# facebookresearch/multimodal

Hardware: NVIDIA H100
Metric: image-text pairs/sec (CLIP ViT-B/16 contrastive pretrain step, bs=512/GPU) (higher is better)
Workload: dtype bf16

## Files before the change

### multimodal_b200/csrc/common.cuh

```cuda
#pragma once
#include <cuda.h>
#include <cuda_bf16.h>
#include <cuda_runtime.h>
#include <stdint.h>
#include <stdio.h>

namespace mmb {

__device__ __forceinline__ uint32_t smem_u32(const void* p) {
  return static_cast<uint32_t>(__cvta_generic_to_shared(p));
}

__device__ __forceinline__ uint64_t global_timer_ns() {
  uint64_t t;
  asm volatile("mov.u64 %0, %%globaltimer;" : "=l"(t));
  return t;
}

#ifndef MMB_WATCHDOG_NS
#define MMB_WATCHDOG_NS 4000000000ull
#endif

__device__ __forceinline__ void mbar_init(uint64_t* bar, uint32_t count) {
  asm volatile("mbarrier.init.shared::cta.b64 [%0], %1;" ::"r"(smem_u32(bar)), "r"(count) : "memory");
// ... 25 lines not shown
      : "=r"(ok)
      : "r"(smem_u32(bar)), "r"(parity)
      : "memory");
  return ok != 0;
}
__device__ __forceinline__ void mbar_wait(uint64_t* bar, uint32_t parity) {
  if (mbar_try_wait(bar, parity)) return;
  uint32_t polls = 0;
  uint64_t t0 = 0;
  while (!mbar_try_wait(bar, parity)) {
#ifdef MMB_WAIT_NANOSLEEP
    __nanosleep(MMB_WAIT_NANOSLEEP);
#endif
    if ((++polls & 1023u) == 0) {
      const uint64_t now = global_timer_ns();
      if (t0 == 0) t0 = now;
      else if (now - t0 > MMB_WATCHDOG_NS) {
        printf("mmb watchdog: mbarrier wait timed out (block %d thread %d parity %u)\n", (int)blockIdx.x,
               (int)threadIdx.x, parity);
        __trap();
      }
    }
  }
}

__device__ __forceinline__ void mbar_wait_quiet(uint64_t* bar, uint32_t parity) {
  if (mbar_try_wait(bar, parity)) return;
  uint32_t polls = 0;
  uint64_t t0 = 0;
  while (!mbar_try_wait(bar, parity)) {
    if ((++polls & 1023u) == 0) {
      const uint64_t now = global_timer_ns();
      if (t0 == 0) t0 = now;
      else if (now - t0 > MMB_WATCHDOG_NS) __trap();
    }
  }
}

__device__ __forceinline__ void tma_prefetch_desc(const CUtensorMap* m) {
  asm volatile("prefetch.tensormap [%0];" ::"l"(reinterpret_cast<uint64_t>(m)) : "memory");
}
__device__ __forceinline__ void tma_prefetch_l2_2d(const CUtensorMap* m, int c0, int c1) {
  asm volatile("cp.async.bulk.prefetch.tensor.2d.L2.global.tile [%0, {%1, %2}];" ::"l"(reinterpret_cast<uint64_t>(m)),
               "r"(c0), "r"(c1)
               : "memory");
}
__device__ __forceinline__ void tma_load_2d(const CUtensorMap* m, uint64_t* bar, void* smem, int c0, int c1) {
  asm volatile(
      "cp.async.bulk.tensor.2d.shared::cluster.global.mbarrier::complete_tx::bytes [%0], [%1, {%3, %4}], [%2];"
      ::"r"(smem_u32(smem)), "l"(reinterpret_cast<uint64_t>(m)), "r"(smem_u32(bar)), "r"(c0), "r"(c1)
      : "memory");
}
__device__ __forceinline__ void tma_load_3d(const CUtensorMap* m, uint64_t* bar, void* smem, int c0, int c1,
                                            int c2) {
  asm volatile(
      "cp.async.bulk.tensor.3d.shared::cluster.global.mbarrier::complete_tx::bytes [%0], [%1, {%3, %4, %5}], [%2];"
      ::"r"(smem_u32(smem)), "l"(reinterpret_cast<uint64_t>(m)), "r"(smem_u32(bar)), "r"(c0), "r"(c1), "r"(c2)
      : "memory");
}
__device__ __forceinline__ void tma_store_2d(const CUtensorMap* m, const void* smem, int c0, int c1) {
  asm volatile("cp.async.bulk.tensor.2d.global.shared::cta.bulk_group [%0, {%2, %3}], [%1];" ::"l"(
                   reinterpret_cast<uint64_t>(m)),
               "r"(smem_u32(smem)), "r"(c0), "r"(c1)
               : "memory");
}
__device__ __forceinline__ void tma_store_3d(const CUtensorMap* m, const void* smem, int c0, int c1, int c2) {
  asm volatile("cp.async.bulk.tensor.3d.global.shared::cta.bulk_group [%0, {%2, %3, %4}], [%1];" ::"l"(
                   reinterpret_cast<uint64_t>(m)),
               "r"(smem_u32(smem)), "r"(c0), "r"(c1), "r"(c2)
               : "memory");
}
__device__ __forceinline__ void tma_reduce_add_2d(const CUtensorMap* m, const void* smem, int c0, int c1) {
  asm volatile("cp.reduce.async.bulk.tensor.2d.global.shared::cta.add.bulk_group [%0, {%2, %3}], [%1];" ::"l"(
                   reinterpret_cast<uint64_t>(m)),
               "r"(smem_u32(smem)), "r"(c0), "r"(c1)
               : "memory");
}
__device__ __forceinline__ void tma_store_commit() { asm volatile("cp.async.bulk.commit_group;" ::: "memory"); }
template <int N>
__device__ __forceinline__ void tma_store_wait_read() {
  asm volatile("cp.async.bulk.wait_group.read %0;" ::"n"(N) : "memory");
}
template <int N>
__device__ __forceinline__ void tma_store_wait_all() {
  asm volatile("cp.async.bulk.wait_group %0;" ::"n"(N) : "memory");
}

__device__ __forceinline__ uint32_t cluster_ctarank() {
  uint32_t r;
  asm volatile("mov.u32 %0, %%cluster_ctarank;" : "=r"(r));
  return r;
}
__device__ __forceinline__ void cluster_sync_all() {
  asm volatile("barrier.cluster.arrive.release.aligned;\n\tbarrier.cluster.wait.acquire.aligned;" ::: "memory");
}
__device__ __forceinline__ void tma_load_2d_multicast(const CUtensorMap* m, uint64_t* bar, void* smem, int c0, int c1,
                                                      uint16_t cta_mask) {
  asm volatile(
      "cp.async.bulk.tensor.2d.shared::cluster.global.mbarrier::complete_tx::bytes.multicast::cluster [%0], [%1, {%3, "
      "%4}], [%2], %5;" ::"r"(smem_u32(smem)),
      "l"(reinterpret_cast<uint64_t>(m)), "r"(smem_u32(bar)), "r"(c0), "r"(c1), "h"(cta_mask)
      : "memory");
}

__device__ __forceinline__ uint64_t make_smem_desc_sw128(uint32_t saddr, uint32_t lbo_bytes, uint32_t sbo_bytes) {
  uint64_t d = 0;
  d |= (uint64_t)((saddr & 0x3FFFFu) >> 4);
  d |= (uint64_t)((lbo_bytes >> 4) & 0x3FFFu) << 16;
  d |= (uint64_t)((sbo_bytes >> 4) & 0x3FFFu) << 32;
  d |= (uint64_t)1 << 62;
  return d;
}
__device__ __forceinline__ void wgmma_fence() { asm volatile("wgmma.fence.sync.aligned;" ::: "memory"); }
__device__ __forceinline__ void wgmma_commit() { asm volatile("wgmma.commit_group.sync.aligned;" ::: "memory"); }
template <int N>
__device__ __forceinline__ void wgmma_wait() {
  asm volatile("wgmma.wait_group.sync.aligned %0;" ::"n"(N) : "memory");
}
template <int TA, int TB>
__device__ __forceinline__ void wgmma_m64n256k16(float (&d)[128], uint64_t adesc, uint64_t bdesc, uint32_t accumulate) {
  asm volatile(
      "{\n\t.reg .pred p;\n\t"
      "setp.ne.b32 p, %130, 0;\n\t"
      "wgmma.mma_async.sync.aligned.m64n256k16.f32.bf16.bf16 "
      "{"
      "%0, %1, %2, %3, %4, %5, %6, %7, %8, %9, %10, %11, %12, %13, %14, %15, "
      "%16, %17, %18, %19, %20, %21, %22, %23, %24, %25, %26, %27, %28, %29, %30, %31, "
      "%32, %33, %34, %35, %36, %37, %38, %39, %40, %41, %42, %43, %44, %45, %46, %47, "
      "%48, %49, %50, %51, %52, %53, %54, %55, %56, %57, %58, %59, %60, %61, %62, %63, "
      "%64, %65, %66, %67, %68, %69, %70, %71, %72, %73, %74, %75, %76, %77, %78, %79, "
      "%80, %81, %82, %83, %84, %85, %86, %87, %88, %89, %90, %91, %92, %93, %94, %95, "
      "%96, %97, %98, %99, %100, %101, %102, %103, %104, %105, %106, %107, %108, %109, %110, %111, "
      "%112, %113, %114, %115, %116, %117, %118, %119, %120, %121, %122, %123, %124, %125, %126, %127"
      "}, %128, %129, p, 1, 1, %131, %132;\n\t}"
      : "+f"(d[0]), "+f"(d[1]), "+f"(d[2]), "+f"(d[3]), "+f"(d[4]), "+f"(d[5]), "+f"(d[6]), "+f"(d[7]),
        "+f"(d[8]), "+f"(d[9]), "+f"(d[10]), "+f"(d[11]), "+f"(d[12]), "+f"(d[13]), "+f"(d[14]), "+f"(d[15]),
        "+f"(d[16]), "+f"(d[17]), "+f"(d[18]), "+f"(d[19]), "+f"(d[20]), "+f"(d[21]), "+f"(d[22]), "+f"(d[23]),
        "+f"(d[24]), "+f"(d[25]), "+f"(d[26]), "+f"(d[27]), "+f"(d[28]), "+f"(d[29]), "+f"(d[30]), "+f"(d[31]),
        "+f"(d[32]), "+f"(d[33]), "+f"(d[34]), "+f"(d[35]), "+f"(d[36]), "+f"(d[37]), "+f"(d[38]), "+f"(d[39]),
        "+f"(d[40]), "+f"(d[41]), "+f"(d[42]), "+f"(d[43]), "+f"(d[44]), "+f"(d[45]), "+f"(d[46]), "+f"(d[47]),
        "+f"(d[48]), "+f"(d[49]), "+f"(d[50]), "+f"(d[51]), "+f"(d[52]), "+f"(d[53]), "+f"(d[54]), "+f"(d[55]),
        "+f"(d[56]), "+f"(d[57]), "+f"(d[58]), "+f"(d[59]), "+f"(d[60]), "+f"(d[61]), "+f"(d[62]), "+f"(d[63]),
        "+f"(d[64]), "+f"(d[65]), "+f"(d[66]), "+f"(d[67]), "+f"(d[68]), "+f"(d[69]), "+f"(d[70]), "+f"(d[71]),
        "+f"(d[72]), "+f"(d[73]), "+f"(d[74]), "+f"(d[75]), "+f"(d[76]), "+f"(d[77]), "+f"(d[78]), "+f"(d[79]),
        "+f"(d[80]), "+f"(d[81]), "+f"(d[82]), "+f"(d[83]), "+f"(d[84]), "+f"(d[85]), "+f"(d[86]), "+f"(d[87]),
        "+f"(d[88]), "+f"(d[89]), "+f"(d[90]), "+f"(d[91]), "+f"(d[92]), "+f"(d[93]), "+f"(d[94]), "+f"(d[95]),
        "+f"(d[96]), "+f"(d[97]), "+f"(d[98]), "+f"(d[99]), "+f"(d[100]), "+f"(d[101]), "+f"(d[102]), "+f"(d[103]),
        "+f"(d[104]), "+f"(d[105]), "+f"(d[106]), "+f"(d[107]), "+f"(d[108]), "+f"(d[109]), "+f"(d[110]), "+f"(d[111]),
        "+f"(d[112]), "+f"(d[113]), "+f"(d[114]), "+f"(d[115]), "+f"(d[116]), "+f"(d[117]), "+f"(d[118]), "+f"(d[119]),
        "+f"(d[120]), "+f"(d[121]), "+f"(d[122]), "+f"(d[123]), "+f"(d[124]), "+f"(d[125]), "+f"(d[126]), "+f"(d[127])
      : "l"(adesc), "l"(bdesc), "r"(accumulate), "n"(TA), "n"(TB));
}

template <int N>
__device__ __forceinline__ void setmaxnreg_dec() { asm volatile("setmaxnreg.dec.sync.aligned.u32 %0;" ::"n"(N)); }
template <int N>
__device__ __forceinline__ void setmaxnreg_inc() { asm volatile("setmaxnreg.inc.sync.aligned.u32 %0;" ::"n"(N)); }

__device__ __forceinline__ void ldsm_x4(uint32_t (&r)[4], uint32_t addr) {
  asm volatile("ldmatrix.sync.aligned.m8n8.x4.shared.b16 {%0,%1,%2,%3}, [%4];"
               : "=r"(r[0]), "=r"(r[1]), "=r"(r[2]), "=r"(r[3])
               : "r"(addr));
}
__device__ __forceinline__ void ldsm_x4_t(uint32_t (&r)[4], uint32_t addr) {
  asm volatile("ldmatrix.sync.aligned.m8n8.x4.trans.shared.b16 {%0,%1,%2,%3}, [%4];"
               : "=r"(r[0]), "=r"(r[1]), "=r"(r[2]), "=r"(r[3])
               : "r"(addr));
}
__device__ __forceinline__ void mma16816(float (&d)[4], const uint32_t (&a)[4], uint32_t b0, uint32_t b1) {
  asm volatile(
      "mma.sync.aligned.m16n8k16.row.col.f32.bf16.bf16.f32 {%0,%1,%2,%3}, {%4,%5,%6,%7}, {%8,%9}, {%0,%1,%2,%3};"
      : "+f"(d[0]), "+f"(d[1]), "+f"(d[2]), "+f"(d[3])
      : "r"(a[0]), "r"(a[1]), "r"(a[2]), "r"(a[3]), "r"(b0), "r"(b1));
}

__device__ __forceinline__ uint32_t pack_bf16x2(float lo, float hi) {
  __nv_bfloat162 v = __floats2bfloat162_rn(lo, hi);
  return *reinterpret_cast<uint32_t*>(&v);
}
__device__ __forceinline__ float bf16_lo(uint32_t v) { return __uint_as_float(v << 16); }
__device__ __forceinline__ float bf16_hi(uint32_t v) { return __uint_as_float(v & 0xFFFF0000u); }

__device__ __forceinline__ float ex2_approx(float x) {
  float y;
  asm("ex2.approx.ftz.f32 %0, %1;" : "=f"(y) : "f"(x));
  return y;
}
__device__ __forceinline__ float rcp_approx(float x) {
  float y;
  asm("rcp.approx.ftz.f32 %0, %1;" : "=f"(y) : "f"(x));
  return y;
}
__device__ __forceinline__ float fast_sigmoid(float z) {
  return rcp_approx(1.f + ex2_approx(-1.4426950408889634f * z));
}
__device__ __forceinline__ float tanh_approx(float x) {
  float y;
  asm("tanh.approx.f32 %0, %1;" : "=f"(y) : "f"(x));
  return y;
}
__device__ __forceinline__ float quick_gelu(float x) {
  const float t = tanh_approx(0.851f * x), h = 0.5f * x;
  return fmaf(h, t, h);
}
__device__ __forceinline__ float quick_gelu_grad(float x) {
  const float u = 0.851f * x;
  const float t = tanh_approx(u);
  return fmaf(0.5f, fmaf(u, fmaf(-t, t, 1.f), t), 0.5f);
}
__device__ __forceinline__ float gelu_erf(float x) { return 0.5f * x * (1.f + erff(x * 0.70710678118654752f)); }
__device__ __forceinline__ float gelu_erf_grad(float x) {
  return 0.5f * (1.f + erff(x * 0.70710678118654752f)) + x * 0.3989422804014327f * ex2_approx(-0.7213475204444817f * x * x);
}
template <int ACT>
__device__ __forceinline__ float act_fn(float x) { return ACT == 0 ? quick_gelu(x) : gelu_erf(x); }
template <int ACT>
__device__ __forceinline__ float act_grad(float x) { return ACT == 0 ? quick_gelu_grad(x) : gelu_erf_grad(x); }

}
```

### multimodal_b200/csrc/gemm.cu

```cuda
#include "common.cuh"
#include "mmb200_internal.h"
#include <stdlib.h>
#include <mutex>

namespace mmb {

constexpr int BLOCK_M = 128;
constexpr int BLOCK_N = 256;
constexpr int BLOCK_K = 64;
constexpr int WG_K = 16;
constexpr int STAGES = 4;
constexpr int A_BYTES = BLOCK_M * BLOCK_K * 2;
constexpr int B_BYTES = BLOCK_N * BLOCK_K * 2;
constexpr int GEMM_THREADS = 384;
constexpr int STG_BYTES = 64 * 128;
constexpr int EPI_SMEM = 4 * STG_BYTES;
constexpr int GEMM_SMEM_BYTES = 1024  + STAGES * (A_BYTES + B_BYTES) + EPI_SMEM + 256 ;
static_assert(GEMM_SMEM_BYTES <= 227 * 1024, "H100: at most 227 KB of shared memory per block");

struct GemmArgs {
  int M, N, K;
  int m_tiles, n_tiles, splits, kb_total, kb_per_split;
  float alpha;
  const float* bias;
// ... 244 lines not shown
            wg_bar_sync(cw);
#pragma unroll
            for (int jj = 0; jj < 4; ++jj) {
              const int j = 4 * q + jj;
              const int n = nq + 8 * j;
              float b0 = 0.f, b1 = 0.f;
              if (add_bias && n < p.N) { b0 = __ldg(p.bias + n); b1 = __ldg(p.bias + n + 1); }
#pragma unroll
              for (int i = 0; i < 2; ++i) {
                const int rr = rl + 8 * i;
                float2* sp = reinterpret_cast<float2*>(buf + rr * 128 + (((2 * jj + (tq >> 1)) ^ (rr & 7)) << 4) + 8 * (tq & 1));
                *sp = make_float2(fmaf(acc[4 * j + 2 * i], p.alpha, b0), fmaf(acc[4 * j + 2 * i + 1], p.alpha, b1));
              }
            }
            fence_proxy_async_smem();
            wg_bar_sync(cw);
            if (elected) {
              if (p.splitk_ws)       tma_store_2d(&tmC0, buf, col0 + 32 * q, split * p.ws_rows + row0);
              else if (p.accumulate) tma_reduce_add_2d(&tmC0, buf, col0 + 32 * q, row0);
              else                   tma_store_2d(&tmC0, buf, col0 + 32 * q, row0);
              tma_store_commit();
            }
            ++stg_next;
          }
        }
      } else {
        float ce_T = 0.f, ce_T2 = 0.f, ce_eps_n = 0.f, ce_gcT = 0.f;
        float ce_lse2[2] = {0.f, 0.f}, ce_gsT[2] = {0.f, 0.f};
        if (EPI == EPI_CE_GRAD) {
          ce_T = __expf(__ldg(p.ce_log_scale));
          ce_T2 = ce_T * 1.4426950408889634f;
          ce_gcT = ce_T * p.ce_gs;
          ce_eps_n = p.ce_smoothing / (float)p.ce_n_total;
#pragma unroll
          for (int i = 0; i < 2; ++i) {
            const int gr = min(r[i], p.M - 1);
            ce_lse2[i] = __ldg(p.ce_lse_row + gr) * 1.4426950408889634f;
            ce_gsT[i] = ce_T * (p.ce_row_w ? p.ce_loss_weight * __ldg(p.ce_row_w + gr) : p.ce_gs);
          }
        }
        const bool do_colsum = (EPI == EPI_BF16 || EPI == EPI_BF16_DACT) && p.colsum_part != nullptr;
        float cs_keep[4][2];
        constexpr int PASSES = EPI == EPI_BF16_ACT ? 2 : 1;
#pragma unroll
        for (int ps = 0; ps < PASSES; ++ps) {
#pragma unroll
          for (int q = 0; q < 4; ++q) {
            cs_keep[q][0] = cs_keep[q][1] = 0.f;
            if (col0 + 64 * q >= p.N) continue;
            const uint32_t b = EPI == EPI_BF16_DACT ? (uint32_t)(q & 1) : (stg_next & 1u);
            uint8_t* buf = stg + b * STG_BYTES;
            if (EPI == EPI_BF16_DACT) {
              mbar_wait_quiet(&aux_bar[2 * cw + b], (aux_phase >> b) & 1u);
              aux_phase ^= 1u << b;
            } else {
              if (elected) tma_store_wait_read<1>();
              wg_bar_sync(cw);
            }
#pragma unroll
            for (int jj = 0; jj < 8; ++jj) {
              const int j = 8 * q + jj;
              const int n = nq + 8 * j;
              const bool col_ok = n < p.N;
              float b0 = 0.f, b1 = 0.f;
              if (add_bias && col_ok) { b0 = __ldg(p.bias + n); b1 = __ldg(p.bias + n + 1); }
              float cs0 = 0.f, cs1 = 0.f;
#pragma unroll
              for (int i = 0; i < 2; ++i) {
                const int rr = rl + 8 * i;
                uint32_t* sp = reinterpret_cast<uint32_t*>(buf + rr * 128 + ((jj ^ (rr & 7)) << 4) + 4 * tq);
                float f0, f1;
                if (EPI == EPI_CE_GRAD) {
                  float f[2];
#pragma unroll
                  for (int e = 0; e < 2; ++e) {
                    const int c = n + e;
                    const float a = acc[4 * j + 2 * i + e];
                    const float tt = ((c == p.ce_label0 + r[i]) ? (1.f - p.ce_smoothing) : 0.f) + ce_eps_n;
                    float gsum = ce_gsT[i] * (ex2_approx(fmaf(a, ce_T2, -ce_lse2[i])) - tt);
                    if (p.ce_lse_col != nullptr && c >= p.ce_col_lo && c < p.ce_col_hi && c < p.N) {
                      const float wc = p.ce_col_w ? p.ce_loss_weight * ce_T * __ldg(p.ce_col_w + c) : ce_gcT;
                      if (wc != 0.f) gsum += wc * (ex2_approx(fmaf(a, ce_T2, -__ldg(p.ce_lse_col + c) * 1.4426950408889634f)) - tt);
                    }
                    f[e] = gsum;
                  }
                  f0 = f[0]; f1 = f[1];
                } else {
                  f0 = fmaf(acc[4 * j + 2 * i], p.alpha, b0);
                  f1 = fmaf(acc[4 * j + 2 * i + 1], p.alpha, b1);
                }
                if (EPI == EPI_BF16_DACT) {
                  const uint32_t av = *sp;
                  f0 *= act_grad<ACT>(bf16_lo(av));
                  f1 *= act_grad<ACT>(bf16_hi(av));
                }
                uint32_t o = pack_bf16x2(f0, f1);
                if (EPI == EPI_BF16_ACT && ps == 1) o = pack_bf16x2(act_fn<ACT>(bf16_lo(o)), act_fn<ACT>(bf16_hi(o)));
                *sp = o;
                if (do_colsum && col_ok && r[i] < p.M) { cs0 += bf16_lo(o); cs1 += bf16_hi(o); }
              }
              if (do_colsum) {
#pragma unroll
                for (int o = 4; o <= 16; o <<= 1) {
                  cs0 += __shfl_xor_sync(0xffffffffu, cs0, o);
                  cs1 += __shfl_xor_sync(0xffffffffu, cs1, o);
                }
                if ((lane >> 2) == jj) { cs_keep[q][0] = cs0; cs_keep[q][1] = cs1; }
              }
            }
            fence_proxy_async_smem();
            wg_bar_sync(cw);
            if (elected) {
              tma_store_2d(EPI == EPI_BF16_ACT && ps == 1 ? &tmC1 : &tmC0, buf, col0 + 64 * q, row0);
              tma_store_commit();
              if (EPI == EPI_BF16_DACT && q + 2 < 4 && col0 + 64 * (q + 2) < p.N) {
                tma_store_wait_read<0>();
                mbar_arrive_expect_tx(&aux_bar[2 * cw + b], STG_BYTES);
                tma_load_2d(&tmC1, &aux_bar[2 * cw + b], buf, col0 + 64 * (q + 2), row0);
              }
            }
            if (EPI != EPI_BF16_DACT) ++stg_next;
          }
        }
        if (do_colsum) {
          if (elected) tma_store_wait_read<0>();
          wg_bar_sync(cw);
          float* sCol = reinterpret_cast<float*>(stg) + wq * BLOCK_N;
#pragma unroll
          for (int q = 0; q < 4; ++q) {
            const int c = 8 * (8 * q + (lane >> 2)) + 2 * tq;
            sCol[c] = cs_keep[q][0];
            sCol[c + 1] = cs_keep[q][1];
          }
          asm volatile("bar.sync 1, 256;" ::: "memory");
          const int ct = threadIdx.x - 128, blk_row = m_blk * TILE_M + (int)rank * BLOCK_M;
          if (blk_row < p.M && col0 + ct < p.N) {
            const float* all = reinterpret_cast<const float*>(sStg);
            float s = 0.f;
#pragma unroll
            for (int w = 0; w < 8; ++w) s += all[(w >> 2) * (2 * STG_BYTES / 4) + (w & 3) * BLOCK_N + ct];
            p.colsum_part[(long long)(blk_row / BLOCK_M) * p.N + col0 + ct] = s;
          }
          fence_proxy_async_smem();
          asm volatile("bar.sync 1, 256;" ::: "memory");
        }
      }
    }
    if (elected) tma_store_wait_all<0>();
  }
  if (CLU) cluster_sync_all();
}
#undef MMB_TILE_SCHEDULE

typedef CUresult (*PFN_encodeTiled)(CUtensorMap*, CUtensorMapDataType, cuuint32_t, void*, const cuuint64_t*,
                                    const cuuint64_t*, const cuuint32_t*, const cuuint32_t*, CUtensorMapInterleave,
                                    CUtensorMapSwizzle, CUtensorMapL2promotion, CUtensorMapFloatOOBfill);

static PFN_encodeTiled get_encode_fn() {
  static PFN_encodeTiled fn = nullptr;
  if (!fn) {
    void* p = nullptr;
    cudaDriverEntryPointQueryResult qres;
    if (cudaGetDriverEntryPoint("cuTensorMapEncodeTiled", &p, cudaEnableDefault, &qres) != cudaSuccess || !p)
      return nullptr;
    fn = reinterpret_cast<PFN_encodeTiled>(p);
  }
  return fn;
}

struct TmapKey {
  const void* ptr; uint64_t inner, outer, pitch; uint32_t box_inner, box_outer, kind;
  bool operator==(const TmapKey& o) const {
    return ptr == o.ptr && inner == o.inner && outer == o.outer && pitch == o.pitch && box_inner == o.box_inner &&
           box_outer == o.box_outer && kind == o.kind;
  }
};
struct TmapSlot { TmapKey key; CUtensorMap map; bool valid; };
constexpr int TMAP_CACHE_SLOTS = 4096;
static TmapSlot* g_tmap_cache = nullptr;
static std::mutex g_tmap_mu;

int make_tmap_2d(CUtensorMap* out, const void* ptr, int elem_bytes, bool is_f32, uint64_t inner, uint64_t outer,
                 uint64_t pitch_bytes, uint32_t box_inner, uint32_t box_outer) {
  PFN_encodeTiled enc = get_encode_fn();
  if (!enc) return MMB_ERR_DRIVER;
  if ((reinterpret_cast<uintptr_t>(ptr) & 15) || (pitch_bytes & 15) || box_inner * elem_bytes != 128) return MMB_ERR_ARG;
  const TmapKey key{ptr, inner, outer, pitch_bytes, box_inner, box_outer, (uint32_t)(is_f32 ? 1 : 0)};
  uint64_t hsh = reinterpret_cast<uintptr_t>(ptr) * 0x9E3779B97F4A7C15ull;
  hsh ^= (inner * 0xC2B2AE3D27D4EB4Full) ^ (outer * 0x165667B19E3779F9ull) ^ (pitch_bytes << 17) ^
         ((uint64_t)box_outer << 40) ^ ((uint64_t)box_inner << 52) ^ key.kind;
  const int slot = (int)((hsh >> 20) % TMAP_CACHE_SLOTS);
  {
    std::lock_guard<std::mutex> lk(g_tmap_mu);
    if (!g_tmap_cache) g_tmap_cache = new TmapSlot[TMAP_CACHE_SLOTS]();
    if (g_tmap_cache[slot].valid && g_tmap_cache[slot].key == key) {
      *out = g_tmap_cache[slot].map;
      return MMB_OK;
    }
  }
  cuuint64_t gdim[2] = {inner, outer};
  cuuint64_t gstr[1] = {pitch_bytes};
  cuuint32_t box[2] = {box_inner, box_outer};
  cuuint32_t estr[2] = {1, 1};
  CUresult r = enc(out, is_f32 ? CU_TENSOR_MAP_DATA_TYPE_FLOAT32 : CU_TENSOR_MAP_DATA_TYPE_BFLOAT16, 2,
                   const_cast<void*>(ptr), gdim, gstr, box, estr, CU_TENSOR_MAP_INTERLEAVE_NONE,
                   CU_TENSOR_MAP_SWIZZLE_128B, CU_TENSOR_MAP_L2_PROMOTION_L2_256B, CU_TENSOR_MAP_FLOAT_OOB_FILL_NONE);
  if (r != CUDA_SUCCESS) return MMB_ERR_DRIVER;
  {
    std::lock_guard<std::mutex> lk(g_tmap_mu);
    g_tmap_cache[slot].key = key;
    g_tmap_cache[slot].map = *out;
    g_tmap_cache[slot].valid = true;
  }
  return MMB_OK;
}

int make_tmap_3d_bf16(CUtensorMap* out, const void* ptr, uint64_t inner, uint64_t dim1, uint64_t dim2, uint64_t pitch1,
                      uint64_t pitch2, uint32_t box_inner, uint32_t box1) {
  PFN_encodeTiled enc = get_encode_fn();
  if (!enc) return MMB_ERR_DRIVER;
  if ((reinterpret_cast<uintptr_t>(ptr) & 15) || (pitch1 & 15) || (pitch2 & 15) || box_inner * 2 != 128) return MMB_ERR_ARG;
  cuuint64_t gdim[3] = {inner, dim1, dim2};
  cuuint64_t gstr[2] = {pitch1, pitch2};
  cuuint32_t box[3] = {box_inner, box1, 1};
  cuuint32_t estr[3] = {1, 1, 1};
  CUresult r = enc(out, CU_TENSOR_MAP_DATA_TYPE_BFLOAT16, 3, const_cast<void*>(ptr), gdim, gstr, box, estr,
                   CU_TENSOR_MAP_INTERLEAVE_NONE, CU_TENSOR_MAP_SWIZZLE_128B, CU_TENSOR_MAP_L2_PROMOTION_L2_256B,
                   CU_TENSOR_MAP_FLOAT_OOB_FILL_NONE);
  return r == CUDA_SUCCESS ? MMB_OK : MMB_ERR_DRIVER;
}

static int g_num_sms = 0;
int num_sms() {
  if (!g_num_sms) {
    int dev = 0;
    cudaGetDevice(&dev);
    cudaDeviceGetAttribute(&g_num_sms, cudaDevAttrMultiProcessorCount, dev);
  }
  return g_num_sms;
}

template <bool A_MN, bool B_MN, int EPI, int ACT, bool CLU>
static int launch_impl(const CUtensorMap& tA, const CUtensorMap& tB, const CUtensorMap& tC0, const CUtensorMap& tC1,
                       const GemmArgs& args, cudaStream_t stream) {
  auto kfn = gemm_kernel<A_MN, B_MN, EPI, ACT, CLU>;
  static bool attr_set = false;
  if (!attr_set) {
    cudaError_t e = cudaFuncSetAttribute(kfn, cudaFuncAttributeMaxDynamicSharedMemorySize, GEMM_SMEM_BYTES);
    if (e != cudaSuccess) return (int)e;
    attr_set = true;
  }
  const int total = args.m_tiles * args.n_tiles * args.splits;
  cudaLaunchConfig_t cfg{};
  cudaLaunchAttribute attr[1];
  if (CLU) {
    const int clusters = total < num_sms() / 2 ? total : num_sms() / 2;
    cfg.gridDim = dim3(2 * clusters);
    attr[0].id = cudaLaunchAttributeClusterDimension;
    attr[0].val.clusterDim.x = 2; attr[0].val.clusterDim.y = 1; attr[0].val.clusterDim.z = 1;
    cfg.attrs = attr; cfg.numAttrs = 1;
  } else {
    cfg.gridDim = dim3(total < num_sms() ? total : num_sms());
  }
  cfg.blockDim = dim3(GEMM_THREADS);
  cfg.dynamicSmemBytes = GEMM_SMEM_BYTES;
  cfg.stream = stream;
  return (int)cudaLaunchKernelEx(&cfg, kfn, tA, tB, tC0, tC1, args);
}

}

using namespace mmb;

static int g_force_cta2 = -1;
extern "C" int mmb_gemm_set_mode(int cta2, int epilogue_warps) {
  if (cta2 < -1 || cta2 > 1 || (epilogue_warps != 0 && epilogue_warps != 8)) return MMB_ERR_ARG;
  g_force_cta2 = cta2;
  return MMB_OK;
}

__global__ void splitk_reduce_kernel(const float* __restrict__ ws, int S, int M, int ws_rows, int N, float* __restrict__ D,
                                     long long ldd, int accumulate) {
  const int n = (blockIdx.x * blockDim.x + threadIdx.x) * 4;
  if (n >= N) return;
  for (int m = blockIdx.y; m < M; m += gridDim.y) {
    float* dst = D + (long long)m * ldd + n;
    float4 acc = accumulate ? make_float4(dst[0], dst[1], dst[2], dst[3]) : make_float4(0.f, 0.f, 0.f, 0.f);
    for (int s = 0; s < S; ++s) {
      const float4 v = *reinterpret_cast<const float4*>(ws + ((long long)s * ws_rows + m) * N + n);
      acc.x += v.x; acc.y += v.y; acc.z += v.z; acc.w += v.w;
    }
    dst[0] = acc.x; dst[1] = acc.y; dst[2] = acc.z; dst[3] = acc.w;
  }
}

static int gemm_launch(int a_mn_major, int b_mn_major, int epilogue, int act, bool cta2, const CUtensorMap& tA,
                       const CUtensorMap& tB, const CUtensorMap& tC0, const CUtensorMap& tC1, const GemmArgs& g,
                       cudaStream_t stream);

static int gemm_dispatch(const void* A, long long lda, int a_mn_major, const void* B, long long ldb, int b_mn_major,
                         void* D0, long long ldd0, void* D1, long long ldd1, int M, int N, int K, int epilogue, int act,
                         float alpha, const float* bias, const void* aux, long long ld_aux, int splits, int accumulate,
                         float* colsum, const GemmArgs* ce, void* stream_) {
  cudaStream_t stream = reinterpret_cast<cudaStream_t>(stream_);
  if (M <= 0 || N <= 0 || K <= 0) return MMB_ERR_ARG;
  if ((epilogue == EPI_CE_STATS || epilogue == EPI_CE_GRAD) && (!ce || a_mn_major || b_mn_major)) return MMB_ERR_ARG;
  if ((lda & 7) || (ldb & 7)) return MMB_ERR_ARG;
  if (epilogue != EPI_CE_STATS && (epilogue == EPI_F32 ? (N & 3) : (N & 7))) return MMB_ERR_ARG;
  const long long big_tiles = (long long)((M + 2 * BLOCK_M - 1) / (2 * BLOCK_M)) * ((N + BLOCK_N - 1) / BLOCK_N);
  const bool cta2 = g_force_cta2 == 1 ||
                    (g_force_cta2 == -1 && M >= 512 && big_tiles * (splits < 1 ? 1 : splits) >= num_sms() / 2);
  GemmArgs g{};
  if (ce) g = *ce;
  g.M = M; g.N = N; g.K = K;
  g.m_tiles = cta2 ? (M + 2 * BLOCK_M - 1) / (2 * BLOCK_M) : (M + BLOCK_M - 1) / BLOCK_M;
  g.n_tiles = (N + BLOCK_N - 1) / BLOCK_N;
  g.kb_total = (K + BLOCK_K - 1) / BLOCK_K;
  if (splits < 1) splits = 1;
  if (splits > g.kb_total) splits = g.kb_total;
  if (epilogue != EPI_F32) splits = 1;
  g.kb_per_split = (g.kb_total + splits - 1) / splits;
  g.splits = (g.kb_total + g.kb_per_split - 1) / g.kb_per_split;
  g.alpha = alpha;
  g.bias = bias;
  g.aux = reinterpret_cast<const __nv_bfloat16*>(aux);
  g.ld_aux = ld_aux;
  g.d0 = D0; g.d1 = D1; g.ldd0 = ldd0; g.ldd1 = ldd1;
  g.accumulate = accumulate ? 1 : 0;
  if (colsum && (epilogue == EPI_F32 || epilogue == EPI_BF16_ACT)) return MMB_ERR_ARG;
  const int col_blocks = (M + BLOCK_M - 1) / BLOCK_M;
  if (colsum) {
    g.colsum_part = static_cast<float*>(scratch(SCR_GEMM_COLSUM, (size_t)col_blocks * N * sizeof(float), stream));
    if (!g.colsum_part) return (int)cudaErrorMemoryAllocation;
  }
  if (epilogue == EPI_F32 && g.splits > 1) {
    g.ws_rows = g.m_tiles * (cta2 ? 2 * BLOCK_M : BLOCK_M);
    g.splitk_ws = static_cast<float*>(scratch(SCR_GEMM_SPLITK, (size_t)g.splits * g.ws_rows * N * sizeof(float), stream));
    if (!g.splitk_ws) return (int)cudaErrorMemoryAllocation;
  }

  CUtensorMap tA, tB;
  int rc;
  if (!a_mn_major) rc = make_tmap_2d(&tA, A, 2, false, K, M, lda * 2, 64, BLOCK_M);
  else             rc = make_tmap_2d(&tA, A, 2, false, M, K, lda * 2, 64, BLOCK_K);
  if (rc) return rc;
  if (!b_mn_major) rc = make_tmap_2d(&tB, B, 2, false, K, N, ldb * 2, 64, cta2 ? BLOCK_N / 2 : BLOCK_N);
  else             rc = make_tmap_2d(&tB, B, 2, false, N, K, ldb * 2, 64, BLOCK_K);
  if (rc) return rc;
  CUtensorMap tC0 = tA, tC1 = tA;
  if (epilogue == EPI_F32) {
    if (ldd0 & 3) return MMB_ERR_ARG;
    if (g.splitk_ws) {
      rc = make_tmap_2d(&tC0, g.splitk_ws, 4, true, N, (uint64_t)g.splits * g.ws_rows, (uint64_t)N * 4, 32, 64);
    } else if ((reinterpret_cast<uintptr_t>(D0) & 15) == 0 && (ldd0 & 3) == 0) {
      rc = make_tmap_2d(&tC0, D0, 4, true, N, M, ldd0 * 4, 32, 64);
    } else {
      g.f32_direct = 1;
    }
    if (rc) return rc;
  } else if (epilogue != EPI_CE_STATS) {
    if ((ldd0 & 7) || (reinterpret_cast<uintptr_t>(D0) & 15)) return MMB_ERR_ARG;
    if (epilogue == EPI_BF16_ACT && (!D1 || (ldd1 & 7) || (reinterpret_cast<uintptr_t>(D1) & 15))) return MMB_ERR_ARG;
    if (epilogue == EPI_BF16_DACT && (!aux || (ld_aux & 7) || (reinterpret_cast<uintptr_t>(aux) & 15))) return MMB_ERR_ARG;
    rc = make_tmap_2d(&tC0, D0, 2, false, N, M, ldd0 * 2, 64, 64);
    if (!rc && epilogue == EPI_BF16_ACT) rc = make_tmap_2d(&tC1, D1, 2, false, N, M, ldd1 * 2, 64, 64);
    if (!rc && epilogue == EPI_BF16_DACT) rc = make_tmap_2d(&tC1, aux, 2, false, N, M, ld_aux * 2, 64, 64);
    if (rc) return rc;
  }

  int rc_launch = gemm_launch(a_mn_major, b_mn_major, epilogue, act, cta2, tA, tB, tC0, tC1, g, stream);
  if (rc_launch) return rc_launch;
  if (g.splitk_ws) {
    splitk_reduce_kernel<<<dim3((N / 4 + 127) / 128, M < 65535 ? M : 65535), 128, 0, stream>>>(
        g.splitk_ws, g.splits, M, g.ws_rows, N, reinterpret_cast<float*>(D0), ldd0, g.accumulate);
    rc_launch = (int)cudaGetLastError();
    if (rc_launch) return rc_launch;
  }
  if (colsum) return reduce_partials(g.colsum_part, col_blocks, N, N, colsum, 1, stream);
  return MMB_OK;
}

static int gemm_launch(int a_mn_major, int b_mn_major, int epilogue, int act, bool cta2, const CUtensorMap& tA,
                       const CUtensorMap& tB, const CUtensorMap& tC0, const CUtensorMap& tC1, const GemmArgs& g,
                       cudaStream_t stream) {
  const int am = a_mn_major ? 1 : 0, bm = b_mn_major ? 1 : 0;
  if (epilogue == EPI_CE_STATS)
    return cta2 ? launch_impl<false, false, EPI_CE_STATS, 0, true>(tA, tB, tC0, tC1, g, stream)
                : launch_impl<false, false, EPI_CE_STATS, 0, false>(tA, tB, tC0, tC1, g, stream);
  if (epilogue == EPI_CE_GRAD)
    return cta2 ? launch_impl<false, false, EPI_CE_GRAD, 0, true>(tA, tB, tC0, tC1, g, stream)
                : launch_impl<false, false, EPI_CE_GRAD, 0, false>(tA, tB, tC0, tC1, g, stream);
#define MMB_CASE(AM, BM, E, AC)                                                                                   \
  if (am == AM && bm == BM && epilogue == E && (AC < 0 || act == AC))                                             \
    return cta2 ? launch_impl<(AM != 0), (BM != 0), E, (AC < 0 ? 0 : AC), true>(tA, tB, tC0, tC1, g, stream)                \
                : launch_impl<(AM != 0), (BM != 0), E, (AC < 0 ? 0 : AC), false>(tA, tB, tC0, tC1, g, stream);
  MMB_CASE(0, 0, EPI_BF16, -1)
  MMB_CASE(0, 0, EPI_BF16_ACT, ACT_QUICK_GELU)
  MMB_CASE(0, 0, EPI_BF16_ACT, ACT_GELU_ERF)
  MMB_CASE(0, 0, EPI_F32, -1)
  MMB_CASE(0, 1, EPI_BF16, -1)
  MMB_CASE(0, 1, EPI_BF16_DACT, ACT_QUICK_GELU)
  MMB_CASE(0, 1, EPI_BF16_DACT, ACT_GELU_ERF)
  MMB_CASE(0, 1, EPI_F32, -1)
  MMB_CASE(1, 1, EPI_F32, -1)
  MMB_CASE(1, 0, EPI_F32, -1)
#undef MMB_CASE
  return MMB_ERR_UNSUPPORTED;
}
extern "C" int mmb_gemm_bf16(const void* A, long long lda, int a_mn_major, const void* B, long long ldb,
                             int b_mn_major, void* D0, long long ldd0, void* D1, long long ldd1, int M, int N, int K,
                             int epilogue, int act, float alpha, const float* bias, const void* aux,
                             long long ld_aux, int splits, int accumulate, float* colsum, void* stream_) {
  if (epilogue < EPI_BF16 || epilogue > EPI_F32) return MMB_ERR_ARG;
  return gemm_dispatch(A, lda, a_mn_major, B, ldb, b_mn_major, D0, ldd0, D1, ldd1, M, N, K, epilogue, act, alpha, bias,
                       aux, ld_aux, splits, accumulate, colsum, nullptr, stream_);
}

extern "C" int mmb_gemm_ce_num_parts(int N) { return N <= 0 ? 0 : (N + 127) / 128; }

static int gemm_ce_stats_impl(const void* A, long long lda, const void* B, long long ldb, int M, int N, int K,
                              const float* log_scale, int label0, const int* labels, void* part, int part_ld, int part0,
                              float* xlabel, void* stream) {
  if (!log_scale || !part || !xlabel || part_ld <= 0 || part0 < 0 || part0 + mmb_gemm_ce_num_parts(N) > part_ld ||
      (reinterpret_cast<uintptr_t>(part) & 15))
    return MMB_ERR_ARG;
  GemmArgs ce{};
  ce.ce_log_scale = log_scale; ce.ce_label0 = label0; ce.ce_labels = labels;
  ce.ce_part = reinterpret_cast<float4*>(part); ce.ce_part_ld = part_ld; ce.ce_part0 = part0; ce.ce_xlabel = xlabel;
  return gemm_dispatch(A, lda, 0, B, ldb, 0, nullptr, 0, nullptr, 0, M, N, K, EPI_CE_STATS, 0, 1.f, nullptr, nullptr, 0, 1, 0,
                       nullptr, &ce, stream);
}

extern "C" int mmb_gemm_ce_stats(const void* A, long long lda, const void* B, long long ldb, int M, int N, int K,
                                 const float* log_scale, int label0, void* part, int part_ld, int part0, float* xlabel,
                                 void* stream) {
  return gemm_ce_stats_impl(A, lda, B, ldb, M, N, K, log_scale, label0, nullptr, part, part_ld, part0, xlabel, stream);
}
extern "C" int mmb_gemm_ce_stats_labels(const void* A, long long lda, const void* B, long long ldb, int M, int N, int K,
                                        const float* log_scale, const int* labels, void* part, int part_ld, int part0,
                                        float* xlabel, void* stream) {
  if (!labels) return MMB_ERR_ARG;
  return gemm_ce_stats_impl(A, lda, B, ldb, M, N, K, log_scale, 0, labels, part, part_ld, part0, xlabel, stream);
}

extern "C" int mmb_gemm_ce_grad(const void* A, long long lda, const void* B, long long ldb, int M, int N, int K,
                                const float* log_scale, int label0, int n_total, int rows_total, float smoothing,
                                float loss_weight, const float* lse_row, const float* row_w, const float* lse_col,
                                const float* col_w, int col_lo, int col_hi, void* dsims_bf16, long long ldd,
                                void* stream) {
  if (!log_scale || !lse_row || !dsims_bf16 || n_total <= 0 || rows_total <= 0) return MMB_ERR_ARG;
  GemmArgs ce{};
  ce.ce_log_scale = log_scale; ce.ce_label0 = label0; ce.ce_n_total = n_total; ce.ce_smoothing = smoothing;
  ce.ce_loss_weight = loss_weight; ce.ce_gs = loss_weight / (float)rows_total;
  ce.ce_lse_row = lse_row; ce.ce_row_w = row_w; ce.ce_lse_col = lse_col; ce.ce_col_w = col_w;
  ce.ce_col_lo = col_lo; ce.ce_col_hi = col_hi;
  return gemm_dispatch(A, lda, 0, B, ldb, 0, dsims_bf16, ldd, nullptr, 0, M, N, K, EPI_CE_GRAD, 0, 1.f, nullptr, nullptr, 0, 1,
                       0, nullptr, &ce, stream);
}
```

Before: 3065.

## Add ping-pong consumer warpgroup GEMM kernel for activation-gradient epilogue

Adds a new 2-CTA cluster GEMM kernel in which the two consumer warpgroups alternate whole output tiles (128x128, N tile narrowed from 256). An order barrier staggers their mainloops so one warpgroup's epilogue (activation-gradient multiply, bias, column-sum, TMA store) overlaps the other's tensor-core mainloop. The kernel uses a new m64n128k16 wgmma wrapper, a 5-stage pipeline and prefetches the aux tile via TMA into the staging buffer. It is enabled by default only for the BF16_DACT epilogue with K-major A and MN-major B. The narrower N tile increases B reloads per output and adds a second register-resident accumulator set per warpgroup.

```diff
diff --git a/multimodal_b200/csrc/common.cuh b/multimodal_b200/csrc/common.cuh
--- a/multimodal_b200/csrc/common.cuh
+++ b/multimodal_b200/csrc/common.cuh
@@ -201,6 +201,29 @@
       : "l"(adesc), "l"(bdesc), "r"(accumulate), "n"(TA), "n"(TB));
 }
 
+template <int TA, int TB>
+__device__ __forceinline__ void wgmma_m64n128k16(float (&d)[64], uint64_t adesc, uint64_t bdesc, uint32_t accumulate) {
+  asm volatile(
+      "{\n\t.reg .pred p;\n\t"
+      "setp.ne.b32 p, %66, 0;\n\t"
+      "wgmma.mma_async.sync.aligned.m64n128k16.f32.bf16.bf16 "
+      "{"
+      "%0, %1, %2, %3, %4, %5, %6, %7, %8, %9, %10, %11, %12, %13, %14, %15, "
+      "%16, %17, %18, %19, %20, %21, %22, %23, %24, %25, %26, %27, %28, %29, %30, %31, "
+      "%32, %33, %34, %35, %36, %37, %38, %39, %40, %41, %42, %43, %44, %45, %46, %47, "
+      "%48, %49, %50, %51, %52, %53, %54, %55, %56, %57, %58, %59, %60, %61, %62, %63"
+      "}, %64, %65, p, 1, 1, %67, %68;\n\t}"
+      : "+f"(d[0]), "+f"(d[1]), "+f"(d[2]), "+f"(d[3]), "+f"(d[4]), "+f"(d[5]), "+f"(d[6]), "+f"(d[7]),
+        "+f"(d[8]), "+f"(d[9]), "+f"(d[10]), "+f"(d[11]), "+f"(d[12]), "+f"(d[13]), "+f"(d[14]), "+f"(d[15]),
+        "+f"(d[16]), "+f"(d[17]), "+f"(d[18]), "+f"(d[19]), "+f"(d[20]), "+f"(d[21]), "+f"(d[22]), "+f"(d[23]),
+        "+f"(d[24]), "+f"(d[25]), "+f"(d[26]), "+f"(d[27]), "+f"(d[28]), "+f"(d[29]), "+f"(d[30]), "+f"(d[31]),
+        "+f"(d[32]), "+f"(d[33]), "+f"(d[34]), "+f"(d[35]), "+f"(d[36]), "+f"(d[37]), "+f"(d[38]), "+f"(d[39]),
+        "+f"(d[40]), "+f"(d[41]), "+f"(d[42]), "+f"(d[43]), "+f"(d[44]), "+f"(d[45]), "+f"(d[46]), "+f"(d[47]),
+        "+f"(d[48]), "+f"(d[49]), "+f"(d[50]), "+f"(d[51]), "+f"(d[52]), "+f"(d[53]), "+f"(d[54]), "+f"(d[55]),
+        "+f"(d[56]), "+f"(d[57]), "+f"(d[58]), "+f"(d[59]), "+f"(d[60]), "+f"(d[61]), "+f"(d[62]), "+f"(d[63])
+      : "l"(adesc), "l"(bdesc), "r"(accumulate), "n"(TA), "n"(TB));
+}
+
 template <int N>
 __device__ __forceinline__ void setmaxnreg_dec() { asm volatile("setmaxnreg.dec.sync.aligned.u32 %0;" ::"n"(N)); }
 template <int N>
diff --git a/multimodal_b200/csrc/gemm.cu b/multimodal_b200/csrc/gemm.cu
--- a/multimodal_b200/csrc/gemm.cu
+++ b/multimodal_b200/csrc/gemm.cu
@@ -420,6 +420,239 @@
 }
 #undef MMB_TILE_SCHEDULE
 
+constexpr int PP_BLOCK_N = 128;
+constexpr int PP_STAGES = 5;
+constexpr int PP_B_BYTES = PP_BLOCK_N * BLOCK_K * 2;
+constexpr int PP_STG_BYTES = 4 * STG_BYTES;
+constexpr int PP_SMEM_BYTES = 1024 + PP_STAGES * (A_BYTES + PP_B_BYTES) + 2 * PP_STG_BYTES + 256;
+static_assert(PP_SMEM_BYTES <= 227 * 1024, "H100: at most 227 KB of shared memory per block");
+
+template <int ACT>
+__global__ void __launch_bounds__(GEMM_THREADS, 1)
+gemm_pingpong_kernel(const __grid_constant__ CUtensorMap tmA, const __grid_constant__ CUtensorMap tmB,
+                     const __grid_constant__ CUtensorMap tmC0, const __grid_constant__ CUtensorMap tmC1,
+                     const GemmArgs p) {
+  extern __shared__ uint8_t smem_raw[];
+  uint8_t* smem = smem_raw + ((1024u - (smem_u32(smem_raw) & 1023u)) & 1023u);
+  uint8_t* sA = smem;
+  uint8_t* sB = smem + PP_STAGES * A_BYTES;
+  uint8_t* sStg = smem + PP_STAGES * (A_BYTES + PP_B_BYTES);
+  uint64_t* full_bar = reinterpret_cast<uint64_t*>(sStg + 2 * PP_STG_BYTES);
+  uint64_t* empty_bar = full_bar + PP_STAGES;
+  uint64_t* aux_bar = empty_bar + PP_STAGES;
+  uint64_t* order_bar = aux_bar + 2;
+  const int wg = threadIdx.x >> 7;
+
+  if (threadIdx.x == 0) {
+    tma_prefetch_desc(&tmA);
+    tma_prefetch_desc(&tmB);
+    for (int i = 0; i < PP_STAGES; ++i) {
+      mbar_init(&full_bar[i], 1);
+      mbar_init(&empty_bar[i], 2);
+    }
+    for (int i = 0; i < 2; ++i) { mbar_init(&aux_bar[i], 1); mbar_init(&order_bar[i], 1); }
+    fence_mbar_init();
+  }
+  cluster_sync_all();
+
+#define MMB_PP_SCHEDULE                                                        \
+  const uint32_t rank = cluster_ctarank();                                     \
+  const int total_tiles = p.m_tiles * p.n_tiles;                               \
+  const int tile_first = (int)(blockIdx.x >> 1), tile_step = (int)(gridDim.x >> 1);
+
+  if (wg == 0) {
+    setmaxnreg_dec<40>();
+    MMB_PP_SCHEDULE
+    if (threadIdx.x == 0) {
+      int stage = 0;
+      uint32_t phase = 0;
+      for (int t = tile_first; t < total_tiles; t += tile_step) {
+        const int m_pair = t / p.n_tiles, n_blk = t - m_pair * p.n_tiles;
+        const int m_blk = 2 * m_pair + (int)rank;
+        const int n0 = n_blk * PP_BLOCK_N;
+        for (int kb = 0; kb < p.kb_total; ++kb) {
+          mbar_wait_quiet(&empty_bar[stage], phase ^ 1);
+          mbar_arrive_expect_tx(&full_bar[stage], A_BYTES + PP_B_BYTES);
+          tma_load_2d(&tmA, &full_bar[stage], sA + stage * A_BYTES, kb * BLOCK_K, m_blk * BLOCK_M);
+          tma_load_2d_multicast(&tmB, &full_bar[stage], sB + stage * PP_B_BYTES + rank * 8192, n0 + (int)rank * 64,
+                                kb * BLOCK_K, 3);
+          if (++stage == PP_STAGES) { stage = 0; phase ^= 1; }
+        }
+      }
+    }
+  } else {
+    setmaxnreg_inc<232>();
+    MMB_PP_SCHEDULE
+    const int cw = wg - 1;
+    const int wq = (threadIdx.x >> 5) & 3;
+    const int lane = threadIdx.x & 31;
+    const int tq = lane & 3;
+    const int rl = wq * 16 + (lane >> 2);
+    const bool elected = (threadIdx.x & 127) == 0;
+    uint8_t* stg = sStg + cw * PP_STG_BYTES;
+    constexpr uint32_t B_KSTEP = (WG_K / 8) * 1024;
+    constexpr uint32_t B_LBO = 64 * BLOCK_K * 2;
+    float acc[2][64];
+    for (int i = cw; tile_first + i * tile_step < total_tiles; i += 2) {
+      const int t = tile_first + i * tile_step;
+      const int m_pair = t / p.n_tiles, n_blk = t - m_pair * p.n_tiles;
+      const int m_blk = 2 * m_pair + (int)rank;
+      const int row0 = m_blk * BLOCK_M;
+      const int col0 = n_blk * PP_BLOCK_N;
+      if (elected) {
+        tma_store_wait_read<0>();
+        const uint32_t bytes = (col0 + 64 < p.N ? 4 : 2) * STG_BYTES;
+        mbar_arrive_expect_tx(&aux_bar[cw], bytes);
+#pragma unroll
+        for (int h = 0; h < 2; ++h)
+#pragma unroll
+          for (int q = 0; q < 2; ++q)
+            if (col0 + 64 * q < p.N)
+              tma_load_2d(&tmC1, &aux_bar[cw], stg + (2 * h + q) * STG_BYTES, col0 + 64 * q, row0 + 64 * h);
+      }
+      if (i > 0) mbar_wait_quiet(&order_bar[cw ^ 1], ((i - 1) >> 1) & 1);
+      const int pos = i * p.kb_total;
+      int stage = pos % PP_STAGES;
+      uint32_t phase = (uint32_t)(pos / PP_STAGES) & 1u;
+      int prev_stage = -1;
+      for (int kb = 0; kb < p.kb_total; ++kb) {
+        mbar_wait_quiet(&full_bar[stage], phase);
+        const uint64_t adesc0 = make_smem_desc_sw128(smem_u32(sA + stage * A_BYTES), 16, 1024);
+        const uint64_t adesc1 = make_smem_desc_sw128(smem_u32(sA + stage * A_BYTES + 8192), 16, 1024);
+        const uint64_t bdesc = make_smem_desc_sw128(smem_u32(sB + stage * PP_B_BYTES), B_LBO, 1024);
+        wgmma_fence();
+#pragma unroll
+        for (int k = 0; k < BLOCK_K / WG_K; ++k) {
+          const uint32_t accum = (kb > 0 || k > 0) ? 1u : 0u;
+          wgmma_m64n128k16<0, 1>(acc[0], adesc0 + (uint64_t)((k * WG_K * 2) >> 4),
+                                            bdesc + (uint64_t)((k * B_KSTEP) >> 4), accum);
+          wgmma_m64n128k16<0, 1>(acc[1], adesc1 + (uint64_t)((k * WG_K * 2) >> 4),
+                                            bdesc + (uint64_t)((k * B_KSTEP) >> 4), accum);
+        }
+        wgmma_commit();
+        wgmma_wait<1>();
+        if (prev_stage >= 0 && elected) {
+          mbar_arrive(&empty_bar[prev_stage]);
+          mbar_arrive_cluster(&empty_bar[prev_stage], rank ^ 1u);
+        }
+        prev_stage = stage;
+        if (++stage == PP_STAGES) { stage = 0; phase ^= 1; }
+      }
+      if (elected) mbar_arrive(&order_bar[cw]);
+      wgmma_wait<0>();
+      if (prev_stage >= 0 && elected) {
+        mbar_arrive(&empty_bar[prev_stage]);
+        mbar_arrive_cluster(&empty_bar[prev_stage], rank ^ 1u);
+      }
+
+      const int nq = col0 + 2 * tq;
+      const bool add_bias = p.bias != nullptr;
+      const bool do_colsum = p.colsum_part != nullptr;
+      float cs_keep[2][2][2];
+      mbar_wait_quiet(&aux_bar[cw], (uint32_t)(i >> 1) & 1u);
+#pragma unroll
+      for (int h = 0; h < 2; ++h) {
+#pragma unroll
+        for (int q = 0; q < 2; ++q) {
+          cs_keep[h][q][0] = cs_keep[h][q][1] = 0.f;
+          if (col0 + 64 * q >= p.N) continue;
+          uint8_t* buf = stg + (2 * h + q) * STG_BYTES;
+          constexpr bool SCATTER = ACT == ACT_QUICK_GELU;
+          const int g = lane >> 2;
+          float cs[8][2], u[4][2], w[2][2];
+#pragma unroll
+          for (int jj = 0; jj < 8; ++jj) {
+            const int j = 8 * q + jj;
+            const int n = nq + 8 * j;
+            const bool col_ok = n < p.N;
+            float b0 = 0.f, b1 = 0.f;
+            if (add_bias && col_ok) { b0 = __ldg(p.bias + n); b1 = __ldg(p.bias + n + 1); }
+            cs[jj][0] = cs[jj][1] = 0.f;
+#pragma unroll
+            for (int ii = 0; ii < 2; ++ii) {
+              const int rr = rl + 8 * ii;
+              uint32_t* sp = reinterpret_cast<uint32_t*>(buf + rr * 128 + ((jj ^ (rr & 7)) << 4) + 4 * tq);
+              const uint32_t av = *sp;
+              const float f0 = fmaf(acc[h][4 * j + 2 * ii], p.alpha, b0) * act_grad<ACT>(bf16_lo(av));
+              const float f1 = fmaf(acc[h][4 * j + 2 * ii + 1], p.alpha, b1) * act_grad<ACT>(bf16_hi(av));
+              const uint32_t o = pack_bf16x2(f0, f1);
+              *sp = o;
+              if (do_colsum && col_ok && row0 + 64 * h + rr < p.M) { cs[jj][0] += bf16_lo(o); cs[jj][1] += bf16_hi(o); }
+            }
+            if (!SCATTER && do_colsum) {
+#pragma unroll
+              for (int e = 0; e < 2; ++e) {
+                float v = cs[jj][e];
+#pragma unroll
+                for (int o = 4; o <= 16; o <<= 1) v += __shfl_xor_sync(0xffffffffu, v, o);
+                if (g == jj) cs_keep[h][q][e] = v;
+              }
+            }
+            if (SCATTER && do_colsum && (jj & 1)) {
+              const int k = jj >> 1;
+              const bool hi = g & 1;
+#pragma unroll
+              for (int e = 0; e < 2; ++e) {
+                const float send = hi ? cs[2 * k][e] : cs[2 * k + 1][e];
+                u[k][e] = (hi ? cs[2 * k + 1][e] : cs[2 * k][e]) + __shfl_xor_sync(0xffffffffu, send, 4);
+              }
+            }
+            if (SCATTER && do_colsum && (jj & 3) == 3) {
+              const int m = jj >> 2;
+              const bool hi = (g >> 1) & 1;
+#pragma unroll
+              for (int e = 0; e < 2; ++e) {
+                const float send = hi ? u[2 * m][e] : u[2 * m + 1][e];
+                w[m][e] = (hi ? u[2 * m + 1][e] : u[2 * m][e]) + __shfl_xor_sync(0xffffffffu, send, 8);
+              }
+            }
+          }
+          if (SCATTER && do_colsum) {
+            const bool hi = (g >> 2) & 1;
+#pragma unroll
+            for (int e = 0; e < 2; ++e) {
+              const float send = hi ? w[0][e] : w[1][e];
+              cs_keep[h][q][e] = (hi ? w[1][e] : w[0][e]) + __shfl_xor_sync(0xffffffffu, send, 16);
+            }
+          }
+          fence_proxy_async_smem();
+          wg_bar_sync(cw);
+          if (elected) {
+            tma_store_2d(&tmC0, buf, col0 + 64 * q, row0 + 64 * h);
+            tma_store_commit();
+          }
+        }
+      }
+      if (do_colsum) {
+        if (elected) tma_store_wait_read<0>();
+        wg_bar_sync(cw);
+        float* sCol = reinterpret_cast<float*>(stg);
+#pragma unroll
+        for (int h = 0; h < 2; ++h)
+#pragma unroll
+          for (int q = 0; q < 2; ++q) {
+            const int c = 8 * (8 * q + (lane >> 2)) + 2 * tq;
+            sCol[(4 * h + wq) * PP_BLOCK_N + c] = cs_keep[h][q][0];
+            sCol[(4 * h + wq) * PP_BLOCK_N + c + 1] = cs_keep[h][q][1];
+          }
+        wg_bar_sync(cw);
+        const int ct = threadIdx.x & 127;
+        if (row0 < p.M && col0 + ct < p.N) {
+          float s = 0.f;
+#pragma unroll
+          for (int w = 0; w < 8; ++w) s += sCol[w * PP_BLOCK_N + ct];
+          p.colsum_part[(long long)m_blk * p.N + col0 + ct] = s;
+        }
+        fence_proxy_async_smem();
+        wg_bar_sync(cw);
+      }
+    }
+    if (elected) tma_store_wait_all<0>();
+  }
+  cluster_sync_all();
+}
+#undef MMB_PP_SCHEDULE
+
 typedef CUresult (*PFN_encodeTiled)(CUtensorMap*, CUtensorMapDataType, cuuint32_t, void*, const cuuint64_t*,
                                     const cuuint64_t*, const cuuint32_t*, const cuuint32_t*, CUtensorMapInterleave,
                                     CUtensorMapSwizzle, CUtensorMapL2promotion, CUtensorMapFloatOOBfill);
@@ -536,6 +769,30 @@
   return (int)cudaLaunchKernelEx(&cfg, kfn, tA, tB, tC0, tC1, args);
 }
 
+template <int ACT>
+static int launch_pingpong(const CUtensorMap& tA, const CUtensorMap& tB, const CUtensorMap& tC0, const CUtensorMap& tC1,
+                           const GemmArgs& args, cudaStream_t stream) {
+  auto kfn = gemm_pingpong_kernel<ACT>;
+  static bool attr_set = false;
+  if (!attr_set) {
+    cudaError_t e = cudaFuncSetAttribute(kfn, cudaFuncAttributeMaxDynamicSharedMemorySize, PP_SMEM_BYTES);
+    if (e != cudaSuccess) return (int)e;
+    attr_set = true;
+  }
+  const int total = args.m_tiles * args.n_tiles;
+  const int clusters = total < num_sms() / 2 ? total : num_sms() / 2;
+  cudaLaunchConfig_t cfg{};
+  cudaLaunchAttribute attr[1];
+  cfg.gridDim = dim3(2 * clusters);
+  attr[0].id = cudaLaunchAttributeClusterDimension;
+  attr[0].val.clusterDim.x = 2; attr[0].val.clusterDim.y = 1; attr[0].val.clusterDim.z = 1;
+  cfg.attrs = attr; cfg.numAttrs = 1;
+  cfg.blockDim = dim3(GEMM_THREADS);
+  cfg.dynamicSmemBytes = PP_SMEM_BYTES;
+  cfg.stream = stream;
+  return (int)cudaLaunchKernelEx(&cfg, kfn, tA, tB, tC0, tC1, args);
+}
+
 }
 
 using namespace mmb;
@@ -566,6 +823,12 @@
                        const CUtensorMap& tB, const CUtensorMap& tC0, const CUtensorMap& tC1, const GemmArgs& g,
                        cudaStream_t stream);
 
+static bool use_pingpong(int a_mn_major, int b_mn_major, int epilogue) {
+  if (g_force_cta2 != -1 || a_mn_major || !b_mn_major || epilogue != EPI_BF16_DACT) return false;
+  const char* e = getenv("MMB_GEMM_PINGPONG");
+  return !(e && e[0] == '0' && e[1] == '\0');
+}
+
 static int gemm_dispatch(const void* A, long long lda, int a_mn_major, const void* B, long long ldb, int b_mn_major,
                          void* D0, long long ldd0, void* D1, long long ldd1, int M, int N, int K, int epilogue, int act,
                          float alpha, const float* bias, const void* aux, long long ld_aux, int splits, int accumulate,
@@ -576,13 +839,14 @@
   if ((lda & 7) || (ldb & 7)) return MMB_ERR_ARG;
   if (epilogue != EPI_CE_STATS && (epilogue == EPI_F32 ? (N & 3) : (N & 7))) return MMB_ERR_ARG;
   const long long big_tiles = (long long)((M + 2 * BLOCK_M - 1) / (2 * BLOCK_M)) * ((N + BLOCK_N - 1) / BLOCK_N);
-  const bool cta2 = g_force_cta2 == 1 ||
-                    (g_force_cta2 == -1 && M >= 512 && big_tiles * (splits < 1 ? 1 : splits) >= num_sms() / 2);
+  const bool pingpong = use_pingpong(a_mn_major, b_mn_major, epilogue);
+  const bool cta2 = !pingpong && (g_force_cta2 == 1 ||
+                    (g_force_cta2 == -1 && M >= 512 && big_tiles * (splits < 1 ? 1 : splits) >= num_sms() / 2));
   GemmArgs g{};
   if (ce) g = *ce;
   g.M = M; g.N = N; g.K = K;
-  g.m_tiles = cta2 ? (M + 2 * BLOCK_M - 1) / (2 * BLOCK_M) : (M + BLOCK_M - 1) / BLOCK_M;
-  g.n_tiles = (N + BLOCK_N - 1) / BLOCK_N;
+  g.m_tiles = cta2 || pingpong ? (M + 2 * BLOCK_M - 1) / (2 * BLOCK_M) : (M + BLOCK_M - 1) / BLOCK_M;
+  g.n_tiles = pingpong ? (N + PP_BLOCK_N - 1) / PP_BLOCK_N : (N + BLOCK_N - 1) / BLOCK_N;
   g.kb_total = (K + BLOCK_K - 1) / BLOCK_K;
   if (splits < 1) splits = 1;
   if (splits > g.kb_total) splits = g.kb_total;
@@ -636,7 +900,12 @@
     if (rc) return rc;
   }
 
-  int rc_launch = gemm_launch(a_mn_major, b_mn_major, epilogue, act, cta2, tA, tB, tC0, tC1, g, stream);
+  int rc_launch;
+  if (pingpong)
+    rc_launch = act == ACT_GELU_ERF ? launch_pingpong<ACT_GELU_ERF>(tA, tB, tC0, tC1, g, stream)
+                                    : launch_pingpong<ACT_QUICK_GELU>(tA, tB, tC0, tC1, g, stream);
+  else
+    rc_launch = gemm_launch(a_mn_major, b_mn_major, epilogue, act, cta2, tA, tB, tC0, tC1, g, stream);
   if (rc_launch) return rc_launch;
   if (g.splitk_ws) {
     splitk_reduce_kernel<<<dim3((N / 4 + 127) / 128, M < 65535 ? M : 65535), 128, 0, stream>>>(
```

After: 3098, median of 6. 1.01x the previous value.
